# toposware/certificate-stark

Hardware: AMD Instinct MI355X
Metric: proofs/sec, state_transition AIR @ 2^20 steps (complete prove(): trace gen, LDE, Blake3 commitments, constraint evaluation, composition, DEEP, FRI, 96 queries) (higher is better)
Workload: dtype u64 (63-bit prime field, Montgomery) + u32 (Blake3)

## Files before the change

certificate-stark_amd/csrc/trace_gen.hip:

```cpp
#include <stdlib.h>
#include "trace_gen.h"
#include "rescue.cuh"
#include "tower.cuh"

namespace cs {

namespace {

constexpr int TXC = 1024;
constexpr int MERKLE_LEN = 512;
constexpr unsigned LADDER_LDS_PAD = 0;
#ifndef CS_RECUR_TILE_ROWS
#define CS_RECUR_TILE_ROWS 16
#endif
#ifndef CS_RECUR_PRIO
#define CS_RECUR_PRIO 3
#endif
constexpr int SCALAR_MUL_LEN = 510;

__device__ __forceinline__ fp mds_row_dot(const fp (&mrow)[14], const fp *xch) {
    Acc128 a = acc_zero();
#pragma unroll
    for (int j = 0; j < 7; j++) acc_mad(a, mrow[j], xch[j]);
    acc_fold(a);
#pragma unroll
    for (int j = 7; j < 14; j++) acc_mad(a, mrow[j], xch[j]);
    acc_fold(a);
    return acc_reduce(a);
}

__device__ __forceinline__ fp rescue_round_lane(fp v, fp *xch, const fp (&mrow)[14], int e, int cyc, bool active) {
    fp x = 0;
    if (active) { x = fp_cube(v); xch[e] = x; }
    __syncthreads();
    if (active) x = fp_inv_sbox(fp_add(mds_row_dot(mrow, xch), c_ark[cyc * 28 + e]));
    __syncthreads();
    if (active) xch[e] = x;
    __syncthreads();
    if (active) v = fp_add(mds_row_dot(mrow, xch), c_ark[cyc * 28 + 14 + e]);
    __syncthreads();
    return v;
}

template <int NCOLS, int LD>
__device__ __forceinline__ void flush_tile(const fp (*tile)[LD], fp *__restrict__ trace, size_t n, size_t row0, int c0, int lane,
                                           int skip_at = -1) {
    for (int c = 0; c < NCOLS; c++) {
        int tc = c0 + c + ((skip_at >= 0 && c >= skip_at) ? 1 : 0);
        trace[(size_t)tc * n + row0 + lane] = tile[lane][c];
    }
}

template <int NCOLS, int LD, int TR>
__device__ __forceinline__ void flush_rows(const fp (*tile)[LD], fp *__restrict__ trace, size_t n, size_t row0, int c0, int lane) {
    for (int c = lane / TR; c < NCOLS; c += 64 / TR) trace[(size_t)(c0 + c) * n + row0 + (lane & (TR - 1))] = tile[lane & (TR - 1)][c];
}

template <bool STANDALONE, int TR>
__global__ __launch_bounds__(64) void k_trace_merkle(TxWitnessDev w, fp *__restrict__ trace, size_t n) {
    __builtin_amdgcn_s_setprio(CS_RECUR_PRIO);
    __shared__ fp tile[TR][65];
    __shared__ fp st[4][14];
    const int t = blockIdx.x, lane = threadIdx.x;
    const int hash_len = 8 * (int)w.depth + 7;
    const bool is_state = lane < 56;
    const int s = is_state ? lane / 14 : 0, e = is_state ? lane % 14 : 0;
    const int col = is_state ? (s == 0 ? 0 : s == 1 ? 15 : s == 2 ? 29 : 44) + e : (lane == 56 ? 14 : lane + 1);
    fp mrow[14];
#pragma unroll
    for (int j = 0; j < 14; j++) mrow[j] = c_mds[e * 14 + j];

    const fp *sv = w.s_old + 14 * (size_t)t, *rv = w.r_old + 14 * (size_t)t;
    const fp delta = w.deltas[t];
    const uint64_t s_index = w.s_idx[t], r_index = w.r_idx[t];
    const fp *s_branch = w.s_paths + (size_t)7 * (w.depth + 1) * t, *r_branch = w.r_paths + (size_t)7 * (w.depth + 1) * t;

    fp v = 0, v2 = 0;
    if (is_state) {
        v = (s < 2 ? sv : rv)[e];
        if (s == 1 && e == 12) v = fp_sub(v, delta);
        if (s == 1 && e == 13) v = fp_add(v, FP_ONE);
        if (s == 3 && e == 12) v = fp_add(v, delta);
    } else if (lane >= 57) {
        v = w.initial_roots[7 * (size_t)t + lane - 57];
    }
    tile[0][col] = v;
    if (lane == 56) tile[0][43] = 0;

    const size_t gbase = (size_t)t * (STANDALONE ? MERKLE_LEN : TXC);
    for (int step = 0; step < MERKLE_LEN - 1; step++) {
        if (step < hash_len) {
            const int cyc = step & 7, lvl = step >> 3;
            if (cyc < 7) {
                v = rescue_round_lane(v, st[s], mrow, e, cyc, is_state);
            } else {
                if (is_state) st[s][e] = v;
                __syncthreads();
                if (is_state) {
                    const fp *node = (s < 2 ? s_branch : r_branch) + 7 * (lvl + 1);
                    const int bit = (int)(((s < 2 ? s_index : r_index) >> lvl) & 1);
                    if (!bit) { if (e >= 7) v = node[e - 7]; }
                    else v = e >= 7 ? st[s][e - 7] : node[e];
                } else if (lane == 56) {
                    v = ((s_index >> lvl) & 1) ? FP_ONE : 0;
                    v2 = ((r_index >> lvl) & 1) ? FP_ONE : 0;
                }
                __syncthreads();
            }
            if (step == hash_len - 1) {
                if (is_state) st[s][e] = v;
                __syncthreads();
                if (lane >= 57) v = st[3][lane - 57];
                __syncthreads();
            }
        }
        const int r = (step + 1) & (TR - 1);
        tile[r][col] = v;
        if (lane == 56) tile[r][43] = v2;
        if (r == TR - 1) {
            __syncthreads();
            flush_rows<65, 65, TR>(tile, trace, n, gbase + (step + 1 - (TR - 1)), 0, lane);
            __syncthreads();
        }
    }
    if (STANDALONE) {
        if (t == 0 && lane == 0) { trace[(size_t)14 * n + 1] = FP_ONE; trace[(size_t)43 * n + 1] = FP_ONE; }
        return;
    }
    if (lane >= 57) st[0][lane - 57] = v;
    __syncthreads();
    for (int k = 0; k < 8; k++)
        for (int c = 58; c < 65; c++) trace[(size_t)c * n + gbase + MERKLE_LEN + 64 * k + lane] = st[0][c - 58];
}

template <bool STANDALONE, int TR>
__global__ __launch_bounds__(64) void k_trace_schnorr_hash(TxWitnessDev w, fp *__restrict__ trace, size_t n) {
    __builtin_amdgcn_s_setprio(CS_RECUR_PRIO);
    __shared__ fp tile[TR][15];
    __shared__ fp st[14];
    const int t = blockIdx.x, lane = threadIdx.x;
    const bool active = lane < 14;
    const int e = active ? lane : 0;
    fp mrow[14];
#pragma unroll
    for (int j = 0; j < 14; j++) mrow[j] = c_mds[e * 14 + j];
    const fp *sv = w.s_old + 14 * (size_t)t, *rv = w.r_old + 14 * (size_t)t;

    fp v = (active && e < 6) ? w.sig_rx[6 * (size_t)t + e] : 0;
    if (active) tile[0][e] = v;
    const size_t gbase = STANDALONE ? (size_t)t * MERKLE_LEN : (size_t)t * TXC + MERKLE_LEN;
    for (int step = 0; step < MERKLE_LEN - 1; step++) {
        if (step < 40) {
            const int cyc = step & 7;
            if (cyc < 7) {
                v = rescue_round_lane(v, st, mrow, e, cyc, active);
            } else if (step < 32) {
                if (active && e >= 7) {
                    int m = 7 * (step >> 3) + e - 7;
                    v = m < 12 ? sv[m] : m < 24 ? rv[m - 12] : m == 24 ? w.deltas[t] : m == 25 ? sv[13] : (STANDALONE ? w.msg_tail[2 * (size_t)t + m - 26] : 0);
                }
            } else {
                if (active && e >= 7) v = 0;
            }
            if (step == 38 && active && e < 4) w.h_limbs[4 * (size_t)t + e] = fp_to_u64(v);
        }
        const int r = (step + 1) & (TR - 1);
        if (active) tile[r][e] = v;
        if (r == TR - 1) {
            __syncthreads();
            flush_rows<14, 15, TR>(tile, trace, n, gbase + (step + 1 - (TR - 1)), 42, lane);
            __syncthreads();
        }
    }
}

struct Term { int8_t slot, coef; };
struct Instr { int8_t out; Term a[3]; Term b[3]; };

enum { SX = 0, SY = 1, SZ = 2, SB3 = 3, SPX = 4, SPY = 5, QX = 27, QY = 28, QZ = 29, NSLOT = 30 };
enum { OP_DOUBLE = 0, OP_ADD_MIXED = 1, OP_ADD_FULL = 2, NPHASE = 6, NROLE = 6 };
#define NOP {-1, {{0, 0}, {0, 0}, {0, 0}}, {{0, 0}, {0, 0}, {0, 0}}}
#define T1(s, c) {{s, c}, {0, 0}, {0, 0}}
#define T2(s, c, s2, c2) {{s, c}, {s2, c2}, {0, 0}}
#define T3(s, c, s2, c2, s3, c3) {{s, c}, {s2, c2}, {s3, c3}}
#define NONE {{0, 0}, {0, 0}, {0, 0}}
#define NOPS6 {NOP, NOP, NOP, NOP, NOP, NOP}
#define CS_EC_PROG { \
     \
    {{{6, T1(0, 1), T1(0, 1)}, {7, T1(1, 1), T1(1, 1)}, {8, T1(2, 1), T1(2, 1)}, {9, T1(0, 1), T1(1, 1)}, {10, T1(0, 1), T1(2, 1)}, {11, T1(1, 1), T1(2, 1)}}, \
     {{12, T1(3, 1), T1(8, 1)}, {13, T1(3, 1), T1(10, 2)}, NOP, NOP, NOP, NOP}, \
     {{19, T3(7, 1, 10, -2, 12, -1), NONE}, {20, T3(7, 1, 10, 2, 12, 1), NONE}, {21, T3(6, 1, 8, -1, 13, 1), NONE}, {22, T2(6, 3, 8, 1), NONE}, NOP, NOP}, \
     {{14, T1(19, 1), T1(20, 1)}, {15, T1(9, 2), T1(19, 1)}, {16, T1(22, 1), T1(21, 1)}, {17, T1(11, 2), T1(21, 1)}, {18, T1(11, 2), T1(7, 1)}, NOP}, \
     {{0, T2(15, 1, 17, -1), NONE}, {1, T2(14, 1, 16, 1), NONE}, {2, T1(18, 4), NONE}, NOP, NOP, NOP}, \
     NOPS6}, \
     \
    {{{6, T1(0, 1), T1(4, 1)}, {7, T1(1, 1), T1(5, 1)}, {8, T1(26, 1), T1(25, 1)}, {9, T1(4, 1), T1(2, 1)}, {10, T1(5, 1), T1(2, 1)}, {11, T1(2, 1), T1(3, 1)}}, \
     {{19, T2(9, 1, 0, 1), NONE}, NOP, NOP, NOP, NOP, NOP}, \
     {{12, T1(19, 1), T1(3, 1)}, NOP, NOP, NOP, NOP, NOP}, \
     {{20, T3(7, 1, 11, -1, 19, -1), NONE}, {21, T3(7, 1, 11, 1, 19, 1), NONE}, {22, T2(6, 3, 2, 1), NONE}, {23, T3(12, 1, 6, 1, 2, -1), NONE}, \
      {24, T2(10, 1, 1, 1), NONE}, {25, T3(8, 1, 6, -1, 7, -1), NONE}}, \
     {{13, T1(20, 1), T1(21, 1)}, {14, T1(22, 1), T1(23, 1)}, {15, T1(24, 1), T1(23, 1)}, {16, T1(25, 1), T1(20, 1)}, {17, T1(25, 1), T1(22, 1)}, {18, T1(24, 1), T1(21, 1)}}, \
     {{0, T2(16, 1, 15, -1), NONE}, {1, T2(13, 1, 14, 1), NONE}, {2, T2(18, 1, 17, 1), NONE}, NOP, NOP, NOP}}, \
     \
    {{{6, T1(0, 1), T1(27, 1)}, {7, T1(1, 1), T1(28, 1)}, {8, T1(2, 1), T1(29, 1)}, {9, T1(20, 1), T1(21, 1)}, {10, T1(22, 1), T1(23, 1)}, {11, T1(24, 1), T1(25, 1)}}, \
     {{19, T3(10, 1, 6, -1, 8, -1), NONE}, NOP, NOP, NOP, NOP, NOP}, \
     {{12, T1(3, 1), T1(8, 1)}, {13, T1(3, 1), T1(19, 1)}, NOP, NOP, NOP, NOP}, \
     {{20, T3(7, 1, 12, -1, 19, -1), NONE}, {21, T3(7, 1, 12, 1, 19, 1), NONE}, {22, T2(6, 3, 8, 1), NONE}, {23, T3(13, 1, 6, 1, 8, -1), NONE}, \
      {24, T3(9, 1, 6, -1, 7, -1), NONE}, {25, T3(11, 1, 7, -1, 8, -1), NONE}}, \
     {{14, T1(20, 1), T1(21, 1)}, {15, T1(22, 1), T1(23, 1)}, {16, T1(25, 1), T1(23, 1)}, {17, T1(24, 1), T1(20, 1)}, {18, T1(24, 1), T1(22, 1)}, {26, T1(25, 1), T1(21, 1)}}, \
     {{0, T2(17, 1, 16, -1), NONE}, {1, T2(14, 1, 15, 1), NONE}, {2, T2(26, 1, 18, 1), NONE}, NOP, NOP, NOP}}, \
}
#define CS_EC_PRE { \
    NOPS6, \
    {{25, T2(0, 1, 1, 1), NONE}, NOP, NOP, NOP, NOP, NOP}, \
    {{20, T2(0, 1, 1, 1), NONE}, {21, T2(27, 1, 28, 1), NONE}, {22, T2(0, 1, 2, 1), NONE}, {23, T2(27, 1, 29, 1), NONE}, {24, T2(1, 1, 2, 1), NONE}, {25, T2(28, 1, 29, 1), NONE}}, \
}
__constant__ Instr c_prog[3][NPHASE][NROLE] = CS_EC_PROG;
__constant__ Instr c_pre[3][NROLE] = CS_EC_PRE;
constexpr Instr k_prog[3][NPHASE][NROLE] = CS_EC_PROG;
constexpr Instr k_pre[3][NROLE] = CS_EC_PRE;
#undef CS_EC_PROG
#undef CS_EC_PRE
constexpr int lin_shape(const Instr (&ph)[NROLE]) {
    int nt = 0, unit = 7;
    for (int m = 0; m < NROLE; m++) {
        if (ph[m].out < 0) continue;
        for (int k = 0; k < 3; k++) {
            const int c = ph[m].a[k].coef;
            if (c != 0 && k + 1 > nt) nt = k + 1;
            if (c < -1 || c > 1) unit &= ~(1 << k);
        }
    }
    return nt | (unit << 4);
}
#undef NOP
#undef T1
#undef T2
#undef T3
#undef NONE
#undef NOPS6

constexpr int8_t PHASE_KIND[3][NPHASE] = {{1, 1, 0, 1, 0, -1}, {1, 0, 1, 0, 1, 0}, {1, 0, 1, 0, 1, 0}};
struct ProgLds { Instr prog[3][NPHASE][NROLE]; Instr pre[3][NROLE]; fp small[9]; };
__device__ __forceinline__ void load_programs(ProgLds &p, int tid, int nthreads) {
    Instr *dst = &p.prog[0][0][0];
    const Instr *src = &c_prog[0][0][0];
    for (int i = tid; i < 3 * NPHASE * NROLE; i += nthreads) dst[i] = src[i];
    for (int i = tid; i < 3 * NROLE; i += nthreads) (&p.pre[0][0])[i] = (&c_pre[0][0])[i];
    if (tid < 9) {
        const int c = tid - 4;
        const fp m = fp_mul((uint64_t)(c < 0 ? -c : c), FP_R2);
        p.small[tid] = c < 0 ? fp_neg(m) : m;
    }
}

template <int SHAPE>
__device__ __forceinline__ Fp2 lincomb2(const fp (*slot)[6], const Term (&t)[3], int comp, const fp *small) {
    Fp2 r = {0, 0};
#pragma unroll
    for (int k = 0; k < (SHAPE & 15); k++) {
        const fp *s = slot[t[k].slot];
        const int cf = t[k].coef;
        fp va, vb;
        if ((SHAPE >> (4 + k)) & 1) {
            va = s[2 * comp]; vb = s[2 * comp + 1];
            if (cf < 0) { va = fp_neg(va); vb = fp_neg(vb); }
            if (cf == 0) { va = 0; vb = 0; }
        } else {
            const fp c = small[cf + 4];
            va = fp_mul(s[2 * comp], c); vb = fp_mul(s[2 * comp + 1], c);
        }
        r = fp2_add(r, {va, vb});
    }
    return r;
}

__device__ __forceinline__ Fp2 operand2(const fp (*slot)[6], const Term t, int comp, int comp2) {
    const fp *s = slot[t.slot];
    Fp2 v = {s[2 * comp], s[2 * comp + 1]};
    if (comp2 >= 0) v = fp2_add(v, {s[2 * comp2], s[2 * comp2 + 1]});
    if (t.coef == 2) v = fp2_dbl(v);
    return v;
}

template <int SHAPE>
__device__ __forceinline__ void run_linear_phase(const Instr (&prog)[NROLE], const fp *small, fp (*slot)[6], int lane, bool enabled) {
    const int m = lane / 3, r = lane % 3;
    Fp2 c = {0, 0};
    int out = -1;
    if (enabled && m < NROLE) {
        const Instr ins = prog[m];
        out = ins.out;
        if (out >= 0) c = lincomb2<SHAPE>(slot, ins.a, r, small);
    }
    __syncthreads();
    if (out >= 0) { slot[out][2 * r] = c.a; slot[out][2 * r + 1] = c.b; }
    __syncthreads();
}

template <int OP, int PH>
__device__ __forceinline__ void run_phases(const ProgLds &pg, fp (*slot)[6], Fp2 (*prod)[6], int lane, bool enabled) {
    if constexpr (PH < NPHASE) {
        if constexpr (PHASE_KIND[OP][PH] >= 0) {
            if constexpr (PHASE_KIND[OP][PH] == 1) {
                const int m = lane / 6, q = lane % 6;
                if (enabled && m < NROLE) {
                    const Instr ins = pg.prog[OP][PH][m];
                    if (ins.out >= 0) {
                        const int c1 = q < 3 ? q : (q == 5 ? 1 : 0), c2 = q < 3 ? -1 : (q == 3 ? 1 : 2);
                        prod[m][q] = fp2_mul(operand2(slot, ins.a[0], c1, c2), operand2(slot, ins.b[0], c1, c2));
                    }
                }
                __syncthreads();
                const int m2 = lane / 3, r = lane % 3;
                if (enabled && m2 < NROLE) {
                    const int out = pg.prog[OP][PH][m2].out;
                    if (out >= 0) {
                        const Fp2 zero = {0, 0};
                        const Fp2 d0 = prod[m2][0], d1 = prod[m2][1], d2 = prod[m2][2];
                        const Fp2 t1 = r == 0 ? d0 : prod[m2][r + 2];
                        const Fp2 t2 = r == 1 ? zero : d1;
                        const Fp2 t3 = r == 0 ? d2 : zero;
                        const Fp2 t4 = r == 2 ? d0 : prod[m2][5];
                        const Fp2 t5 = r == 0 ? zero : (r == 1 ? d0 : fp2_dbl(d2));
                        const Fp2 c = fp2_sub(fp2_sub(fp2_add(fp2_add(t1, t2), t3), t4), t5);
                        slot[out][2 * r] = c.a;
                        slot[out][2 * r + 1] = c.b;
                    }
                }
                __syncthreads();
            } else {
                run_linear_phase<lin_shape(k_prog[OP][PH])>(pg.prog[OP][PH], pg.small, slot, lane, enabled);
            }
            run_phases<OP, PH + 1>(pg, slot, prod, lane, enabled);
        }
    }
}
template <int OP>
__device__ __forceinline__ void run_point_op(const ProgLds &pg, fp (*slot)[6], Fp2 (*prod)[6], int lane, bool enabled) {
    if constexpr (OP != OP_DOUBLE) run_linear_phase<lin_shape(k_pre[OP])>(pg.pre[OP], pg.small, slot, lane, enabled);
    run_phases<OP, 0>(pg, slot, prod, lane, enabled);
}

__device__ __forceinline__ int bit_le(const uint8_t *bytes, int i) { return (bytes[i >> 3] >> (i & 7)) & 1; }

template <bool STANDALONE, int TR>
__global__ __launch_bounds__(64) void k_trace_schnorr_ec(TxWitnessDev w, fp *__restrict__ trace, size_t n) {
    __builtin_amdgcn_s_setprio(CS_RECUR_PRIO);
    constexpr int TG = 64 / TR;
    __shared__ fp tile[TR][19];
    __shared__ fp slots[NSLOT][6];
    __shared__ Fp2 prods[6][6];
    __shared__ uint8_t sbytes[32];
    __shared__ ProgLds pg;
    const int t = blockIdx.x >> 1, g = blockIdx.x & 1, lane = threadIdx.x;
    fp(*slot)[6] = slots;
    load_programs(pg, lane, 64);

    if (lane < 32) sbytes[lane] = g == 0 ? w.sig_s[32 * (size_t)t + lane] : (uint8_t)(w.h_limbs[4 * (size_t)t + (lane >> 3)] >> (8 * (lane & 7)));
    if (lane < 6) {
        slot[SX][lane] = 0;
        slot[SY][lane] = lane == 0 ? FP_ONE : 0;
        slot[SZ][lane] = 0;
        slot[SB3][lane] = c_b3[lane];
        slot[SPX][lane] = g == 0 ? c_generator[lane] : w.s_old[14 * (size_t)t + lane];
        slot[SPY][lane] = g == 0 ? c_generator[6 + lane] : w.s_old[14 * (size_t)t + 6 + lane];
        slot[26][lane] = fp_add(slot[SPX][lane], slot[SPY][lane]);
    }
    __syncthreads();
    if (lane < 18) tile[0][lane] = slot[lane / 6][lane % 6];
    const size_t gbase = STANDALONE ? (size_t)t * MERKLE_LEN : (size_t)t * TXC + MERKLE_LEN;

    for (int step = 0; step < MERKLE_LEN - 1; step++) {
        if (step < SCALAR_MUL_LEN) {
            if ((step & 1) == 0) {
                run_point_op<OP_DOUBLE>(pg, slot, prods, lane, true);
            } else {
                const int bit = bit_le(sbytes, 254 - (step >> 1));
                if (bit) run_point_op<OP_ADD_MIXED>(pg, slot, prods, lane, true);
            }
        }
        const int r = (step + 1) & (TR - 1);
        if (lane < 18) tile[r][lane] = slot[lane / 6][lane % 6];
        if (r == TR - 1) {
            __syncthreads();
            for (int c = lane / TR; c < 18; c += TG) trace[(size_t)(g * 19 + c) * n + gbase + (step + 1 - (TR - 1)) + (lane & (TR - 1))] = tile[lane & (TR - 1)][c];
            __syncthreads();
        }
    }
}
template <bool STANDALONE>
__global__ __launch_bounds__(64) void k_trace_schnorr_final(fp *__restrict__ trace, size_t n) {
    __shared__ fp slots[NSLOT][6];
    __shared__ Fp2 prods[6][6];
    __shared__ ProgLds pg;
    const int t = blockIdx.x, lane = threadIdx.x;
    load_programs(pg, lane, 64);
    const size_t last = (STANDALONE ? (size_t)t * MERKLE_LEN : (size_t)t * TXC + MERKLE_LEN) + MERKLE_LEN - 1;
    if (lane < 18) {
        slots[lane / 6][lane % 6] = trace[(size_t)lane * n + last - 1];
        slots[QX + lane / 6][lane % 6] = trace[(size_t)(19 + lane) * n + last - 1];
    }
    if (lane < 6) slots[SB3][lane] = c_b3[lane];
    __syncthreads();
    run_point_op<OP_ADD_FULL>(pg, slots, prods, lane, true);
    if (lane == 0) fp6_store(slots[SX], fp6_mul(fp6_load(slots[SX]), fp6_inv(fp6_load(slots[SZ]))));
    __syncthreads();
    if (lane < 18) trace[(size_t)lane * n + last] = slots[lane / 6][lane % 6];
}

__device__ __forceinline__ fp small_to_fp(uint64_t x) { return fp_mul(x, FP_R2); }

template <int WHICH>
__global__ __launch_bounds__(256) void k_trace_aux(TxWitnessDev w, fp *__restrict__ trace, size_t n) {
    constexpr bool PLAIN = WHICH != 2, WITH_H = WHICH != 1;
    const int t = blockIdx.x;
    const int r = blockIdx.y * 256 + threadIdx.x;
    const size_t g = (size_t)t * TXC + r;
    const fp *sv = w.s_old + 14 * (size_t)t, *rv = w.r_old + 14 * (size_t)t;
    const fp delta = w.deltas[t];
    const fp sigma = fp_sub(sv[12], delta);
    if (PLAIN) {
        for (int i = 0; i < 12; i++) {
            trace[(size_t)(65 + i) * n + g] = sv[i];
            trace[(size_t)(77 + i) * n + g] = rv[i];
        }
        trace[(size_t)89 * n + g] = delta;
        trace[(size_t)90 * n + g] = sigma;
        trace[(size_t)91 * n + g] = sv[13];
    }
    if (r < MERKLE_LEN) {
        if (PLAIN) {
            trace[(size_t)92 * n + g] = 0;
            trace[(size_t)93 * n + g] = 0;
        }
        return;
    }
    const int q = r - MERKLE_LEN;
    const uint64_t dv = fp_to_u64(delta), sg = fp_to_u64(sigma);
    if (PLAIN) {
        const int k = q < 64 ? q : 64;
        uint64_t dacc = k == 0 ? 0 : dv >> (64 - k), sacc = k == 0 ? 0 : sg >> (64 - k);
        trace[(size_t)56 * n + g] = (dacc & 1) ? FP_ONE : 0;
        trace[(size_t)57 * n + g] = small_to_fp(dacc);
        trace[(size_t)92 * n + g] = (sacc & 1) ? FP_ONE : 0;
        trace[(size_t)93 * n + g] = small_to_fp(sacc);
    }
    const uint8_t *sb = w.sig_s + 32 * (size_t)t;
    const uint64_t *h = w.h_limbs + 4 * (size_t)t;
    fp bs = 0, bh = 0;
    if (q >= 1) {
        const int step = q - 1 < SCALAR_MUL_LEN - 1 ? q - 1 : SCALAR_MUL_LEN - 1;
        const int bi = 254 - (step >> 1);
        bs = bit_le(sb, bi) ? FP_ONE : 0;
        bh = ((h[bi >> 6] >> (bi & 63)) & 1) ? FP_ONE : 0;
        if (q == SCALAR_MUL_LEN + 1) bs = FP_ONE;
    }
    if (PLAIN) trace[(size_t)18 * n + g] = bs;
    if (!WITH_H) return;
    trace[(size_t)37 * n + g] = bh;
    const int k = (q + 1) / 2 < 255 ? (q + 1) / 2 : 255;
    for (int c = 0; c < 4; c++) {
        const int width = c == 0 ? 63 : 64;
        const int start = c == 0 ? 0 : 63 + 64 * (c - 1);
        int kc = k - start;
        kc = kc < 0 ? 0 : kc > width ? width : kc;
        const uint64_t limb = h[3 - c];
        const uint64_t acc = kc == 0 ? 0 : (c == 0 ? (limb >> (63 - kc)) : (kc == 64 ? limb : limb >> (64 - kc)));
        trace[(size_t)(41 - c) * n + g] = small_to_fp(acc);
    }
}

}

static unsigned ladder_lds_pad() {
    static const unsigned pad = [] { const char *e = getenv("CSTARK_EC_LDS_PAD"); return e ? (unsigned)atoi(e) : LADDER_LDS_PAD; }();
    return pad;
}
hipError_t launch_trace_gen(const TxWitnessDev &w, fp *d_trace, hipStream_t stream, hipStream_t side, hipEvent_t fork, hipEvent_t join) {
    const size_t n = (size_t)w.n_tx * TXC;
    hipError_t e;
    if ((e = hipEventRecord(fork, stream)) != hipSuccess) return e;
    if ((e = hipStreamWaitEvent(side, fork, 0)) != hipSuccess) return e;
    hipLaunchKernelGGL((k_trace_merkle<false, 64>), dim3(w.n_tx), dim3(64), 0, side, w, d_trace, n);
    if ((e = hipEventRecord(join, side)) != hipSuccess) return e;
    hipLaunchKernelGGL((k_trace_schnorr_hash<false, 64>), dim3(w.n_tx), dim3(64), 0, stream, w, d_trace, n);
    hipLaunchKernelGGL((k_trace_schnorr_ec<false, 64>), dim3(2 * w.n_tx), dim3(64), 0, stream, w, d_trace, n);
    hipLaunchKernelGGL(k_trace_schnorr_final<false>, dim3(w.n_tx), dim3(64), 0, stream, d_trace, n);
    hipLaunchKernelGGL(k_trace_aux<0>, dim3(w.n_tx, 4), dim3(256), 0, stream, w, d_trace, n);
    if ((e = hipStreamWaitEvent(stream, join, 0)) != hipSuccess) return e;
    return hipGetLastError();
}

hipError_t launch_trace_gen_split(const TxWitnessDev &w, fp *d_trace, hipStream_t stream, hipStream_t side_a, hipStream_t side_b, hipEvent_t fork,
                                  hipEvent_t join_a, hipEvent_t mid_b, hipEvent_t join_b) {
    const size_t n = (size_t)w.n_tx * TXC;
    hipError_t e;
    if ((e = hipEventRecord(fork, stream)) != hipSuccess) return e;
    hipLaunchKernelGGL(k_trace_aux<1>, dim3(w.n_tx, 4), dim3(256), 0, stream, w, d_trace, n);
    if ((e = hipStreamWaitEvent(side_a, fork, 0)) != hipSuccess) return e;
    if ((e = hipStreamWaitEvent(side_b, fork, 0)) != hipSuccess) return e;
    hipLaunchKernelGGL((k_trace_merkle<false, CS_RECUR_TILE_ROWS>), dim3(w.n_tx), dim3(64), 0, side_a, w, d_trace, n);
    if ((e = hipEventRecord(join_a, side_a)) != hipSuccess) return e;
    hipLaunchKernelGGL((k_trace_schnorr_hash<false, CS_RECUR_TILE_ROWS>), dim3(w.n_tx), dim3(64), 0, side_b, w, d_trace, n);
    hipLaunchKernelGGL(k_trace_aux<2>, dim3(w.n_tx, 4), dim3(256), 0, side_b, w, d_trace, n);
    if ((e = hipEventRecord(mid_b, side_b)) != hipSuccess) return e;
    static const int ec_rows = [] { const char *e = getenv("CSTARK_EC_TILE_ROWS"); return e ? atoi(e) : 16; }();
    if (ec_rows == 64) hipLaunchKernelGGL((k_trace_schnorr_ec<false, 64>), dim3(2 * w.n_tx), dim3(64), ladder_lds_pad(), side_b, w, d_trace, n);
    else if (ec_rows == 32) hipLaunchKernelGGL((k_trace_schnorr_ec<false, 32>), dim3(2 * w.n_tx), dim3(64), ladder_lds_pad(), side_b, w, d_trace, n);
    else hipLaunchKernelGGL((k_trace_schnorr_ec<false, 16>), dim3(2 * w.n_tx), dim3(64), ladder_lds_pad(), side_b, w, d_trace, n);
    hipLaunchKernelGGL(k_trace_schnorr_final<false>, dim3(w.n_tx), dim3(64), 0, side_b, d_trace, n);
    if ((e = hipEventRecord(join_b, side_b)) != hipSuccess) return e;
    return hipGetLastError();
}

__global__ __launch_bounds__(256) void k_trace_schnorr_bits(TxWitnessDev w, fp *__restrict__ trace, size_t n) {
    const int t = blockIdx.x;
    const int q = blockIdx.y * 256 + threadIdx.x;
    const size_t g = (size_t)t * MERKLE_LEN + q;
    const uint8_t *sb = w.sig_s + 32 * (size_t)t;
    const uint64_t *h = w.h_limbs + 4 * (size_t)t;
    fp bs = 0, bh = 0;
    if (q >= 1) {
        const int step = q - 1 < SCALAR_MUL_LEN - 1 ? q - 1 : SCALAR_MUL_LEN - 1;
        const int bi = 254 - (step >> 1);
        bs = bit_le(sb, bi) ? FP_ONE : 0;
        bh = ((h[bi >> 6] >> (bi & 63)) & 1) ? FP_ONE : 0;
        if (q == SCALAR_MUL_LEN + 1) bs = FP_ONE;
    }
    trace[(size_t)18 * n + g] = bs;
    trace[(size_t)37 * n + g] = bh;
    const int k = (q + 1) / 2 < 255 ? (q + 1) / 2 : 255;
    for (int c = 0; c < 4; c++) {
        const int width = c == 0 ? 63 : 64, start = c == 0 ? 0 : 63 + 64 * (c - 1);
        int kc = k - start;
        kc = kc < 0 ? 0 : kc > width ? width : kc;
        const uint64_t limb = h[3 - c];
        const uint64_t acc = kc == 0 ? 0 : (c == 0 ? (limb >> (63 - kc)) : (kc == 64 ? limb : limb >> (64 - kc)));
        trace[(size_t)(41 - c) * n + g] = small_to_fp(acc);
    }
}
__global__ __launch_bounds__(256) void k_schnorr_aux_columns(TxWitnessDev w, fp *__restrict__ out, size_t n) {
    const int t = blockIdx.x;
    const int q = blockIdx.y * 256 + threadIdx.x;
    const size_t g = (size_t)t * MERKLE_LEN + q;
    const fp *sv = w.s_old + 14 * (size_t)t, *rv = w.r_old + 14 * (size_t)t;
    for (int j = 0; j < 12; j++) out[(size_t)j * n + g] = sv[j];
    const bool chunk_row = q < 32 && (q & 7) == 7;
    for (int j = 0; j < 7; j++) {
        fp v = 0;
        if (chunk_row) {
            const int m = j + 7 * (q >> 3);
            v = m < 12 ? sv[m] : m < 24 ? rv[m - 12] : m == 24 ? w.deltas[t] : m == 25 ? sv[13] : w.msg_tail[2 * (size_t)t + m - 26];
        }
        out[(size_t)(12 + j) * n + g] = v;
    }
}
hipError_t launch_schnorr_trace(const TxWitnessDev &w, fp *d_trace, hipStream_t stream) {
    const size_t n = (size_t)w.n_tx * MERKLE_LEN;
    hipLaunchKernelGGL((k_trace_schnorr_hash<true, 64>), dim3(w.n_tx), dim3(64), 0, stream, w, d_trace, n);
    hipLaunchKernelGGL((k_trace_schnorr_ec<true, 64>), dim3(2 * w.n_tx), dim3(64), 0, stream, w, d_trace, n);
    hipLaunchKernelGGL(k_trace_schnorr_final<true>, dim3(w.n_tx), dim3(64), 0, stream, d_trace, n);
    hipLaunchKernelGGL(k_trace_schnorr_bits, dim3(w.n_tx, 2), dim3(256), 0, stream, w, d_trace, n);
    return hipGetLastError();
}
hipError_t launch_schnorr_trace_split(const TxWitnessDev &w, fp *d_trace, hipStream_t stream, hipStream_t side, hipEvent_t fork, hipEvent_t join_a,
                                      hipEvent_t join_b) {
    const size_t n = (size_t)w.n_tx * MERKLE_LEN;
    hipError_t e;
    if ((e = hipEventRecord(fork, stream)) != hipSuccess) return e;
    if ((e = hipStreamWaitEvent(side, fork, 0)) != hipSuccess) return e;
    hipLaunchKernelGGL((k_trace_schnorr_hash<true, 64>), dim3(w.n_tx), dim3(64), 0, side, w, d_trace, n);
    hipLaunchKernelGGL(k_trace_schnorr_bits, dim3(w.n_tx, 2), dim3(256), 0, side, w, d_trace, n);
    if ((e = hipEventRecord(join_a, side)) != hipSuccess) return e;
    if (w.n_tx <= 512) hipLaunchKernelGGL((k_trace_schnorr_ec<true, 64>), dim3(2 * w.n_tx), dim3(64), 0, side, w, d_trace, n);
    else hipLaunchKernelGGL((k_trace_schnorr_ec<true, 16>), dim3(2 * w.n_tx), dim3(64), 0, side, w, d_trace, n);
    hipLaunchKernelGGL(k_trace_schnorr_final<true>, dim3(w.n_tx), dim3(64), 0, side, d_trace, n);
    if ((e = hipEventRecord(join_b, side)) != hipSuccess) return e;
    return hipGetLastError();
}
hipError_t launch_schnorr_aux_columns(const TxWitnessDev &w, fp *d_out, hipStream_t stream) {
    const size_t n = (size_t)w.n_tx * MERKLE_LEN;
    hipLaunchKernelGGL(k_schnorr_aux_columns, dim3(w.n_tx, 2), dim3(256), 0, stream, w, d_out, n);
    return hipGetLastError();
}

struct RescueSeed { fp s[7]; };
__global__ __launch_bounds__(64) void k_trace_rescue_chain(RescueSeed seed, fp *__restrict__ trace, size_t n) {
    __shared__ fp tile[64][15];
    __shared__ fp xch[14];
    const int lane = threadIdx.x, e = lane < 14 ? lane : 0;
    const bool active = lane < 14;
    fp mrow[14];
#pragma unroll
    for (int j = 0; j < 14; j++) mrow[j] = c_mds[e * 14 + j];
    fp v = (active && lane < 7) ? seed.s[lane] : 0;
    if (active) tile[0][e] = v;
    for (size_t step = 0; step + 1 < n; step++) {
        const int cyc = (int)(step & 7);
        if (cyc < 7) v = rescue_round_lane(v, xch, mrow, e, cyc, active);
        else if (lane >= 7) v = 0;
        const int r = (int)((step + 1) & 63);
        if (active) tile[r][e] = v;
        if (r == 63) {
            __syncthreads();
            for (int c = 0; c < 14; c++) trace[(size_t)c * n + (step + 1 - 63) + lane] = tile[lane][c];
            __syncthreads();
        }
    }
}
hipError_t launch_rescue_chain_trace(const uint64_t seed[7], unsigned iterations, fp *d_trace, hipStream_t stream) {
    RescueSeed s;
    for (int i = 0; i < 7; i++) s.s[i] = seed[i];
    hipLaunchKernelGGL(k_trace_rescue_chain, dim3(1), dim3(64), 0, stream, s, d_trace, (size_t)iterations * 8);
    return hipGetLastError();
}

hipError_t launch_merkle_trace(const TxWitnessDev &w, fp *d_trace, hipStream_t stream) {
    const size_t n = (size_t)w.n_tx * MERKLE_LEN;
    hipLaunchKernelGGL((k_trace_merkle<true, 64>), dim3(w.n_tx), dim3(64), 0, stream, w, d_trace, n);
    return hipGetLastError();
}

__global__ void k_trace_range(uint64_t number, fp *trace) {
    const int q = threadIdx.x;
    const uint64_t v63 = number & 0x7FFFFFFFFFFFFFFFULL;
    const uint64_t acc = q == 0 ? 0 : v63 >> (63 - q);
    trace[q] = (q >= 1 && (acc & 1)) ? FP_ONE : 0;
    trace[64 + q] = fp_from_u64(acc);
}
hipError_t launch_range_trace(uint64_t number_canonical, fp *d_trace, hipStream_t stream) {
    hipLaunchKernelGGL(k_trace_range, dim3(1), dim3(64), 0, stream, number_canonical, d_trace);
    return hipGetLastError();
}

__global__ __launch_bounds__(256) void k_range_chunk_prefix(const uint64_t *__restrict__ words, fp *__restrict__ prefix, unsigned n_chunks) {
    __shared__ fp seg[256], lead[256];
    const unsigned t = threadIdx.x, per = (n_chunks + 255) / 256, c0 = t * per, c1 = min(c0 + per, n_chunks);
    const fp B = FP_R2;
    fp v = 0;
    for (unsigned c = c0; c < c1; c++) v = fp_add(fp_mul(v, B), fp_from_u64(words[n_chunks - 1 - c]));
    seg[t] = v;
    __syncthreads();
    if (t == 0) {
        const fp Bper = fp_pow(B, per);
        fp carry = 0;
        for (unsigned i = 0; i < 256; i++) { lead[i] = carry; carry = fp_add(fp_mul(carry, Bper), seg[i]); }
    }
    __syncthreads();
    v = lead[t];
    for (unsigned c = c0; c < c1; c++) { v = fp_add(fp_mul(v, B), fp_from_u64(words[n_chunks - 1 - c])); prefix[c] = v; }
}
__global__ __launch_bounds__(256) void k_trace_range_bits(const uint64_t *__restrict__ words, const fp *__restrict__ prefix, fp *__restrict__ trace,
                                                          unsigned log_n) {
    const size_t n = (size_t)1 << log_n, q = blockIdx.x * (size_t)256 + threadIdx.x;
    if (q >= n) return;
    const unsigned c = (unsigned)(q >> 6), r = (unsigned)(q & 63), n_chunks = (unsigned)(n >> 6);
    const uint64_t u = words[n_chunks - 1 - c];
    const fp before = c ? prefix[c - 1] : 0;
    const fp two_r1 = fp_pow(fp_from_u64(2), r + 1);
    trace[q] = ((u >> (63 - r)) & 1) ? FP_ONE : 0;
    trace[n + q] = fp_add(fp_mul(before, two_r1), fp_from_u64(u >> (63 - r)));
}
hipError_t launch_range_trace_bits(const uint64_t *d_words, fp *d_prefix, fp *d_trace, unsigned log_n, hipStream_t stream) {
    const size_t n = (size_t)1 << log_n;
    hipLaunchKernelGGL(k_range_chunk_prefix, dim3(1), dim3(256), 0, stream, d_words, d_prefix, (unsigned)(n >> 6));
    hipLaunchKernelGGL(k_trace_range_bits, dim3((unsigned)((n + 255) / 256)), dim3(256), 0, stream, d_words, (const fp *)d_prefix, d_trace, log_n);
    return hipGetLastError();
}

}
```

Baseline: 39.97.

## Pack ten EC scalar-mul ladders per wavefront with bit-masked mixed adds

Replaces the one-ladder-per-block Schnorr EC trace kernel with a packed kernel that runs ten ladders in one 64-lane block, six lanes per ladder, sharing the LDS program and tile buffers. Point ops are specialised at compile time on coefficient masks so small-coefficient scaling only emits the multiples that are used. Mixed adds run when any ladder in the group has the bit set, and only ladders whose bit is set commit the result. This cuts idle lanes and block count in the serial ladder, at the cost of more LDS per block and some wasted adds for ladders whose bit is zero.

```diff
diff --git a/certificate-stark_amd/csrc/trace_gen.hip b/certificate-stark_amd/csrc/trace_gen.hip
--- a/certificate-stark_amd/csrc/trace_gen.hip
+++ b/certificate-stark_amd/csrc/trace_gen.hip
@@ -9,7 +9,6 @@
 
 constexpr int TXC = 1024;
 constexpr int MERKLE_LEN = 512;
-constexpr unsigned LADDER_LDS_PAD = 0;
 #ifndef CS_RECUR_TILE_ROWS
 #define CS_RECUR_TILE_ROWS 16
 #endif
@@ -389,6 +388,171 @@
         }
     }
 }
+constexpr int PK_LAD = 10;
+constexpr int PK_TR = 16;
+
+constexpr int coef_mask(const Instr (&ph)[NROLE], int k, bool B) {
+    int mask = 0;
+    for (int m = 0; m < NROLE; m++) {
+        if (ph[m].out < 0) continue;
+        const int c = B ? ph[m].b[k].coef : ph[m].a[k].coef;
+        mask |= (1 << (c < 0 ? -c : c)) | (c < 0 ? 256 : 0);
+    }
+    return mask;
+}
+template <int MASK>
+__device__ __forceinline__ fp scale_small(fp v, int acf) {
+    fp r = v;
+    if constexpr ((MASK & 0x1c) != 0) {
+        const fp v2 = fp_dbl(v);
+        if (acf == 2) r = v2;
+        if constexpr ((MASK & 8) != 0) { const fp v3 = fp_add(v2, v); if (acf == 3) r = v3; }
+        if constexpr ((MASK & 16) != 0) { const fp v4 = fp_dbl(v2); if (acf == 4) r = v4; }
+    }
+    if constexpr ((MASK & 1) != 0) { if (acf == 0) r = 0; }
+    return r;
+}
+template <int MASK>
+__device__ __forceinline__ Fp6 operand6(const fp (*slot)[6], const Term t) {
+    Fp6 v = fp6_load(slot[t.slot]);
+    if constexpr ((MASK & 0xfd) != 0) {
+#pragma unroll
+        for (int i = 0; i < 6; i++) v.c[i] = scale_small<MASK>(v.c[i], t.coef);
+    }
+    return v;
+}
+template <int M0, int M1, int M2>
+__device__ __forceinline__ void packed_linear_phase(const Instr (&prog)[NROLE], fp (*slot)[6], int m, bool has_role, bool commit) {
+    Fp6 c = {{0, 0, 0, 0, 0, 0}};
+    int out = -1;
+    if (has_role) {
+        const Instr ins = prog[m];
+        out = ins.out;
+        if (out >= 0) {
+            constexpr int MASKS[3] = {M0, M1, M2};
+            bool have = false;
+#pragma unroll
+            for (int k = 0; k < 3; k++) {
+                if ((MASKS[k] & 0xfe) == 0) continue;
+                const fp *s = slot[ins.a[k].slot];
+                const int cf = ins.a[k].coef, acf = cf < 0 ? -cf : cf;
+#pragma unroll
+                for (int i = 0; i < 6; i++) {
+                    fp v = k == 0 ? scale_small<M0>(s[i], acf) : k == 1 ? scale_small<M1>(s[i], acf) : scale_small<M2>(s[i], acf);
+                    if ((MASKS[k] & 256) != 0 && cf < 0) v = fp_neg(v);
+                    c.c[i] = have ? fp_add(c.c[i], v) : v;
+                }
+                have = true;
+            }
+        }
+    }
+    __syncthreads();
+    if (out >= 0 && commit) fp6_store(slot[out], c);
+    __syncthreads();
+}
+template <int OP, int PH>
+__device__ __forceinline__ void packed_phases(const ProgLds &pg, fp (*slot)[6], int m, bool has_role, bool commit) {
+    if constexpr (PH < NPHASE) {
+        if constexpr (PHASE_KIND[OP][PH] >= 0) {
+            if constexpr (PHASE_KIND[OP][PH] == 1) {
+                int out = -1;
+                Fp6 r = {{0, 0, 0, 0, 0, 0}};
+                if (has_role) {
+                    const Instr ins = pg.prog[OP][PH][m];
+                    out = ins.out;
+                    if (out >= 0)
+                        r = fp6_mul(operand6<coef_mask(k_prog[OP][PH], 0, false)>(slot, ins.a[0]),
+                                    operand6<coef_mask(k_prog[OP][PH], 0, true)>(slot, ins.b[0]));
+                }
+                __syncthreads();
+                if (out >= 0) fp6_store(slot[out], r);
+                __syncthreads();
+            } else {
+                constexpr bool LAST = PH + 1 == NPHASE || PHASE_KIND[OP][PH + 1 < NPHASE ? PH + 1 : PH] < 0;
+                packed_linear_phase<coef_mask(k_prog[OP][PH], 0, false), coef_mask(k_prog[OP][PH], 1, false), coef_mask(k_prog[OP][PH], 2, false)>(
+                    pg.prog[OP][PH], slot, m, has_role, LAST ? commit : true);
+            }
+            packed_phases<OP, PH + 1>(pg, slot, m, has_role, commit);
+        }
+    }
+}
+template <int OP>
+__device__ __forceinline__ void packed_point_op(const ProgLds &pg, fp (*slot)[6], int m, bool has_role, bool commit) {
+    if constexpr (OP != OP_DOUBLE)
+        packed_linear_phase<coef_mask(k_pre[OP], 0, false), coef_mask(k_pre[OP], 1, false), coef_mask(k_pre[OP], 2, false)>(pg.pre[OP], slot, m,
+                                                                                                                         has_role, true);
+    packed_phases<OP, 0>(pg, slot, m, has_role, commit);
+}
+
+__global__ __launch_bounds__(64) void k_trace_schnorr_ec_packed(TxWitnessDev w, fp *__restrict__ trace, size_t n) {
+    __builtin_amdgcn_s_setprio(CS_RECUR_PRIO);
+    constexpr int TR = PK_TR, TG = 64 / TR;
+    __shared__ fp tile[PK_LAD][TR][19];
+    __shared__ fp slots[PK_LAD][NSLOT][6];
+    __shared__ uint8_t sbytes[PK_LAD + 1][32];
+    __shared__ ProgLds pg;
+    const int lane = threadIdx.x;
+    const int n_lad = 2 * (int)w.n_tx;
+    const bool has_role = lane < 6 * PK_LAD;
+    const int l = has_role ? lane / 6 : 0, m = lane % 6;
+    const int lad0 = PK_LAD * (int)blockIdx.x;
+    fp(*slot)[6] = slots[l];
+    load_programs(pg, lane, 64);
+
+    for (int i = lane; i < PK_LAD * 32; i += 64) {
+        const int gl = lad0 + i / 32, b = i % 32, t = gl >> 1;
+        uint8_t v = 0;
+        if (gl < n_lad) v = (gl & 1) == 0 ? w.sig_s[32 * (size_t)t + b] : (uint8_t)(w.h_limbs[4 * (size_t)t + (b >> 3)] >> (8 * (b & 7)));
+        sbytes[i / 32][b] = v;
+    }
+    if (has_role) {
+        const int gl = lad0 + l, t = gl >> 1;
+        const bool own_key = gl < n_lad && (gl & 1) != 0;
+        slot[SX][m] = 0;
+        slot[SY][m] = m == 0 ? FP_ONE : 0;
+        slot[SZ][m] = 0;
+        slot[SB3][m] = c_b3[m];
+        const fp px = own_key ? w.s_old[14 * (size_t)t + m] : c_generator[m];
+        const fp py = own_key ? w.s_old[14 * (size_t)t + 6 + m] : c_generator[6 + m];
+        slot[SPX][m] = px;
+        slot[SPY][m] = py;
+        slot[26][m] = fp_add(px, py);
+    }
+    __syncthreads();
+    if (lane < 32) {
+        uint8_t any = 0;
+        for (int k = 0; k < PK_LAD; k++) any |= sbytes[k][lane];
+        sbytes[PK_LAD][lane] = any;
+    }
+    if (has_role)
+        for (int j = 0; j < 3; j++) tile[l][0][6 * j + m] = slot[j][m];
+    __syncthreads();
+
+    for (int step = 0; step < MERKLE_LEN - 1; step++) {
+        if (step < SCALAR_MUL_LEN) {
+            if ((step & 1) == 0) {
+                packed_point_op<OP_DOUBLE>(pg, slot, m, has_role, true);
+            } else {
+                const int bi = 254 - (step >> 1);
+                const int any = __builtin_amdgcn_readfirstlane(bit_le(sbytes[PK_LAD], bi));
+                if (any) packed_point_op<OP_ADD_MIXED>(pg, slot, m, has_role, bit_le(sbytes[l], bi) != 0);
+            }
+        }
+        const int r = (step + 1) & (TR - 1);
+        if (has_role)
+            for (int j = 0; j < 3; j++) tile[l][r][6 * j + m] = slot[j][m];
+        if (r == TR - 1) {
+            __syncthreads();
+            const size_t row0 = (size_t)(step + 1 - (TR - 1)) + (lane & (TR - 1));
+            for (int i = lane / TR; i < PK_LAD * 18; i += TG) {
+                const int fl = i / 18, c = i % 18, gl = lad0 + fl, t = gl >> 1;
+                if (gl >= n_lad) break;
+                trace[(size_t)((gl & 1) * 19 + c) * n + (size_t)t * TXC + MERKLE_LEN + row0] = tile[fl][lane & (TR - 1)][c];
+            }
+            __syncthreads();
+        }
+    }
+}
 template <bool STANDALONE>
 __global__ __launch_bounds__(64) void k_trace_schnorr_final(fp *__restrict__ trace, size_t n) {
     __shared__ fp slots[NSLOT][6];
@@ -473,10 +637,7 @@
 
 }
 
-static unsigned ladder_lds_pad() {
-    static const unsigned pad = [] { const char *e = getenv("CSTARK_EC_LDS_PAD"); return e ? (unsigned)atoi(e) : LADDER_LDS_PAD; }();
-    return pad;
-}
+static dim3 packed_grid(uint32_t n_tx) { return dim3((2 * n_tx + PK_LAD - 1) / PK_LAD); }
 hipError_t launch_trace_gen(const TxWitnessDev &w, fp *d_trace, hipStream_t stream, hipStream_t side, hipEvent_t fork, hipEvent_t join) {
     const size_t n = (size_t)w.n_tx * TXC;
     hipError_t e;
@@ -485,7 +646,7 @@
     hipLaunchKernelGGL((k_trace_merkle<false, 64>), dim3(w.n_tx), dim3(64), 0, side, w, d_trace, n);
     if ((e = hipEventRecord(join, side)) != hipSuccess) return e;
     hipLaunchKernelGGL((k_trace_schnorr_hash<false, 64>), dim3(w.n_tx), dim3(64), 0, stream, w, d_trace, n);
-    hipLaunchKernelGGL((k_trace_schnorr_ec<false, 64>), dim3(2 * w.n_tx), dim3(64), 0, stream, w, d_trace, n);
+    hipLaunchKernelGGL(k_trace_schnorr_ec_packed, packed_grid(w.n_tx), dim3(64), 0, stream, w, d_trace, n);
     hipLaunchKernelGGL(k_trace_schnorr_final<false>, dim3(w.n_tx), dim3(64), 0, stream, d_trace, n);
     hipLaunchKernelGGL(k_trace_aux<0>, dim3(w.n_tx, 4), dim3(256), 0, stream, w, d_trace, n);
     if ((e = hipStreamWaitEvent(stream, join, 0)) != hipSuccess) return e;
@@ -505,10 +666,7 @@
     hipLaunchKernelGGL((k_trace_schnorr_hash<false, CS_RECUR_TILE_ROWS>), dim3(w.n_tx), dim3(64), 0, side_b, w, d_trace, n);
     hipLaunchKernelGGL(k_trace_aux<2>, dim3(w.n_tx, 4), dim3(256), 0, side_b, w, d_trace, n);
     if ((e = hipEventRecord(mid_b, side_b)) != hipSuccess) return e;
-    static const int ec_rows = [] { const char *e = getenv("CSTARK_EC_TILE_ROWS"); return e ? atoi(e) : 16; }();
-    if (ec_rows == 64) hipLaunchKernelGGL((k_trace_schnorr_ec<false, 64>), dim3(2 * w.n_tx), dim3(64), ladder_lds_pad(), side_b, w, d_trace, n);
-    else if (ec_rows == 32) hipLaunchKernelGGL((k_trace_schnorr_ec<false, 32>), dim3(2 * w.n_tx), dim3(64), ladder_lds_pad(), side_b, w, d_trace, n);
-    else hipLaunchKernelGGL((k_trace_schnorr_ec<false, 16>), dim3(2 * w.n_tx), dim3(64), ladder_lds_pad(), side_b, w, d_trace, n);
+    hipLaunchKernelGGL(k_trace_schnorr_ec_packed, packed_grid(w.n_tx), dim3(64), 0, side_b, w, d_trace, n);
     hipLaunchKernelGGL(k_trace_schnorr_final<false>, dim3(w.n_tx), dim3(64), 0, side_b, d_trace, n);
     if ((e = hipEventRecord(join_b, side_b)) != hipSuccess) return e;
     return hipGetLastError();
```

Result: no change. 39.90 (median of 2 runs) (-0.2%).
